# LiliMeng/network_interpretation_imagenet

Measured on AMD Instinct MI355X. Metric: masked-forward-passes/sec (224x224, resnet101), higher is better.
Workload: dtype f16x3 (split-fp16 MFMA, fp32 accumulate); stem conv in fp32 by superposition over superpixels; 1 GPU; resnet101, 512 masks/image x 128 images per GPU (BASELINE configs[2]; x1 GPUs); images_per_gpu=128, masks_per_image=512, forward_batch=2340, num_cus=256, entry=MaskedForwardEngine.score_packed, stem=table, lib_stamp=5d2f2b6c2eede968ac8309a9a3169fc2d6f530e9f9ea7d38be715b004f9c220a, lib_stamp_matches_tree=True, product_library=True, parallelism=mask-batch shard x1 + one all_gather of scores

## Files before the change

### include/mpx.h

```cpp
#ifndef MPX_H
#define MPX_H

#include <stddef.h>
#include <stdint.h>

#ifdef __cplusplus
extern "C" {
#endif

#define MPX_IMG 224
#define MPX_IMG_PAD 230
#define MPX_NUM_CLASSES 1000

enum {
    MPX_E_ARG = -1,
    MPX_E_STATE = -2,
    MPX_E_NOMEM = -3,
    MPX_E_INTERNAL = -4
};

#define MPX_ARCH_MNIST_NET 1
#define MPX_ARCH_CIFAR_RESNET 2000
#define MPX_ARCH_VGG 3000
#define MPX_ARCH_VGG_BN 3100
// ... 50 lines not shown
    int32_t hin;
    int32_t clamp_in;
} mpx_dwconv_desc;
int mpx_num_dwconvs(const mpx_engine* h);
int mpx_dwconv_info(const mpx_engine* h, int k, mpx_dwconv_desc* out);
int mpx_load_dwconv(mpx_engine* h, int k, const float* w, const float* gamma, const float* beta, const float* mean, const float* var, float eps);
int mpx_dwconv_params(const mpx_engine* h, int k, const float** w, const float** scale, const float** shift);

int mpx_set_conv_tile(mpx_engine* h, int i, int tile);
int mpx_get_conv_tile(const mpx_engine* h, int i);
int mpx_last_conv_kernels(const mpx_engine* h);

int mpx_pack_conv_weights(const mpx_conv_desc* d, const float* w, const float* conv_bias, const float* gamma,
                          const float* beta, const float* mean, const float* var, float eps,
                          uint16_t* w_hi, uint16_t* w_lo, float* scale, float* shift);
int mpx_mask_apply_normalize(mpx_engine* h, const uint8_t* img_u8_hwc, const float* img_f32_chw,
                             const int32_t* seg, const uint8_t* onoff, int M, int S,
                             const float mean[3], const float std[3], int slot0,
                             float* out_f32_nchw, void* stream);

int mpx_stem_table_build(mpx_engine* h, const uint8_t* img_u8_hwc, const float* img_f32_chw, const int32_t* seg, int S,
                         const float mean[3], const float std[3], void* stream);
int mpx_stem_table_apply(mpx_engine* h, const uint8_t* onoff, int M, int S, int slot0, void* stream);

int mpx_mask_apply_minmax(mpx_engine* h, const float* img_f32_chw, const int32_t* seg, const uint8_t* removed,
                          int M, int S, int slot0, float* out_f32_nchw, void* stream);

int mpx_avgpool2_pad(mpx_engine* h, const void* in_hi, const void* in_lo, void* out_hi, void* out_lo, int B,
                     int hin, int cin_p, int cout_p, void* stream);

int mpx_conv_bn_act(mpx_engine* h, int i, const void* in_hi, const void* in_lo,
                    const void* res_hi, const void* res_lo, void* out_hi, void* out_lo,
                    float* out_f32, int B, void* stream);

int mpx_conv_dual_bn_act(mpx_engine* h, int i, const void* in_hi, const void* in_lo, const void* x_hi,
                         const void* x_lo, void* out_hi, void* out_lo, int B, void* stream);
int mpx_set_fusion(mpx_engine* h, int mask);

int mpx_bottleneck_tail(mpx_engine* h, int i, const void* t1_hi, const void* t1_lo, const void* x_hi, const void* x_lo,
                        void* out_hi, void* out_lo, void* next_hi, void* next_lo, int B, void* stream);
int mpx_num_bottleneck_tails(const mpx_engine* h);
int mpx_bottleneck_tail_info(const mpx_engine* h, int k, int* conv2, int* conv3, int* downsample, int* next_conv1);

int mpx_maxpool3x3s2(mpx_engine* h, const void* in_hi, const void* in_lo, void* out_hi,
                     void* out_lo, int B, int hin, int c, void* stream);

// ... 60 lines not shown
```

### network_interpretation_imagenet_amd/_lib.py

```python
import ctypes as C
import os

import torch

_HERE = os.path.dirname(os.path.abspath(__file__))
PRODUCT_LIB_PATH = os.path.join(_HERE, "libmpx.so")
LIB_PATH = os.environ.get("MPX_LIB_PATH") or PRODUCT_LIB_PATH

IMG = 224
IMG_PAD = 230
NUM_CLASSES = 1000


class MpxError(RuntimeError):
    pass


class ConvDesc(C.Structure):
    _fields_ = [("name", C.c_char * 48), ("bn_name", C.c_char * 48),
                ("cin", C.c_int32), ("cout", C.c_int32), ("ksize", C.c_int32),
                ("stride", C.c_int32), ("pad", C.c_int32), ("hin", C.c_int32),
                ("hout", C.c_int32), ("relu", C.c_int32), ("residual", C.c_int32),
                ("k_packed", C.c_int32), ("cout_pad", C.c_int32)]

# ... 11 lines not shown
_fp = C.POINTER(C.c_float)

SIGNATURES = {
    "mpx_create": (_i, [_i, _i, _i, C.POINTER(_vp)]),
    "mpx_destroy": (_i, [_vp]),
    "mpx_last_error": (C.c_char_p, [_vp]),
    "mpx_max_batch": (_i, [_vp]),
    "mpx_num_cus": (_i, [_vp]),
    "mpx_workspace_bytes": (C.c_size_t, [_vp]),
    "mpx_num_convs": (_i, [_vp]),
    "mpx_conv_info": (_i, [_vp, _i, C.POINTER(ConvDesc)]),
    "mpx_set_conv_weights": (_i, [_vp, _i, _vp, _vp, _vp, _vp, _vp, _vp, _f]),
    "mpx_geometry": (_i, [_vp, C.POINTER(_i), C.POINTER(_i), C.POINTER(_i), C.POINTER(_i)]),
    "mpx_mask_apply_minmax": (_i, [_vp, _vp, _vp, _vp, _i, _i, _i, _vp, _vp]),
    "mpx_avgpool2_pad": (_i, [_vp, _vp, _vp, _vp, _vp, _i, _i, _i, _i, _vp]),
    "mpx_weights_complete": (_i, [_vp]),
    "mpx_set_conv_tile": (_i, [_vp, _i, _i]),
    "mpx_get_conv_tile": (_i, [_vp, _i]),
    "mpx_last_conv_kernels": (_i, [_vp]),
    "mpx_pack_conv_weights": (_i, [C.POINTER(ConvDesc), _vp, _vp, _vp, _vp, _vp, _vp, _f, _vp, _vp, _vp, _vp]),
    "mpx_mask_apply_normalize": (_i, [_vp, _vp, _vp, _vp, _vp, _i, _i, _fp, _fp, _i, _vp, _vp]),
    "mpx_stem_table_build": (_i, [_vp, _vp, _vp, _vp, _i, _fp, _fp, _vp]),
    "mpx_stem_table_apply": (_i, [_vp, _vp, _i, _i, _i, _vp]),
    "mpx_conv_bn_act": (_i, [_vp, _i, _vp, _vp, _vp, _vp, _vp, _vp, _vp, _i, _vp]),
    "mpx_conv_dual_bn_act": (_i, [_vp, _i, _vp, _vp, _vp, _vp, _vp, _vp, _i, _vp]),
    "mpx_set_fusion": (_i, [_vp, _i]),
    "mpx_bottleneck_tail": (_i, [_vp, _i, _vp, _vp, _vp, _vp, _vp, _vp, _vp, _vp, _i, _vp]),
    "mpx_num_bottleneck_tails": (_i, [_vp]),
    "mpx_bottleneck_tail_info": (_i, [_vp, _i, C.POINTER(_i), C.POINTER(_i), C.POINTER(_i), C.POINTER(_i)]),
    "mpx_stem_conv_maxpool": (_i, [_vp, _vp, _vp, _i, _vp]),
    "mpx_maxpool3x3s2": (_i, [_vp, _vp, _vp, _vp, _vp, _i, _i, _i, _vp]),
    "mpx_maxpool2x2s2": (_i, [_vp, _vp, _vp, _vp, _vp, _i, _i, _i, _vp]),
    "mpx_maxpool3x3s2p0": (_i, [_vp, _vp, _vp, _vp, _vp, _i, _i, _i, _vp]),
    "mpx_global_avgpool": (_i, [_vp, _vp, _vp, _vp, _vp, _i, _i, _i, _vp]),
    "mpx_head_softmax_gather": (_i, [_vp, _vp, _vp, _vp, _vp, _i, _vp]),
    "mpx_forward": (_i, [_vp, _vp, _vp, _vp, _vp, _i, _vp]),
    "mpx_heatmap_accumulate": (_i, [_vp, _vp, _vp, _vp, _vp, _i, _i, _vp, _vp]),
    "mpx_input_planes": (_i, [_vp, C.POINTER(_vp), C.POINTER(_vp)]),
    "mpx_mark_input_staged": (_i, [_vp, _i, _i]),
    "mpx_stem_planes": (_i, [_vp, C.POINTER(_vp), C.POINTER(_vp)]),
    "mpx_profile_enable": (_i, [_vp, _i]),
    "mpx_profile_collect": (_i, [_vp, C.POINTER(C.c_double), C.POINTER(C.c_longlong), C.POINTER(C.c_double)]),
    "mpx_flops_per_forward": (C.c_double, [_vp]),
    "mpx_num_norms": (_i, [_vp]),
    "mpx_norm_info": (_i, [_vp, _i, C.POINTER(NormDesc)]),
    "mpx_load_norm": (_i, [_vp, _i, _vp, _vp, _vp, _vp, _f]),
# ... 66 lines not shown
```

### network_interpretation_imagenet_amd/csrc/mpx_api.hip

```cpp
#include "../../include/mpx.h"
#include "mpx_kernels.h"
#include "mpx_conv3p.h"
#include "mpx_conv3pp.h"
#include "mpx_conv256.h"
#include "mpx_conv256p.h"
#include "mpx_convx.h"
#include "mpx_convw.h"
#include "mpx_btail.h"
#include "mpx_stemtab.h"
#include "mpx_dw.h"
#include "mpx_fire.h"
#include "mpx_pool3c.h"

#include <algorithm>
#include <cmath>
#include <cstdarg>
#include <initializer_list>
#include <new>
#include <cstdio>
#include <cstdlib>
#include <cstring>
#include <string>
#include <vector>

// ... 118 lines not shown
    char* arena = nullptr;
    size_t arena_bytes = 0;
    char* tab_arena = nullptr;
    size_t tab_arena_bytes = 0;
    half_t* in_hi = nullptr;
    half_t* in_lo = nullptr;
    half_t* act_hi[kActBufs] = {};
    half_t* act_lo[kActBufs] = {};
    half_t* pool_hi = nullptr;
    half_t* pool_lo = nullptr;
    float* logits = nullptr;
    float* seg_scratch = nullptr;
    half_t* stem_hi = nullptr;
    half_t* stem_lo = nullptr;
    float* stem_w32 = nullptr;
    float* stem_s32 = nullptr;
    float* stem_t32 = nullptr;
    int* tab_cnt = nullptr;
    int* tab_off = nullptr;
    int* tab_lab = nullptr;
    int* tab_heavy = nullptr;
    float* tab_vec = nullptr;
    unsigned* tab_bits = nullptr;
    size_t tab_sizes[4] = {0, 0, 0, 0};
    int tab_S = -1;
    bool stem_w_loaded = false;
    std::vector<uint8_t> slot_src;
    std::string err;
    bool in_forward = false;
    unsigned last_kernels = 0;
    bool fuse_ds = true;
    bool fuse_pool = true;
    bool prof_on = false;
    std::vector<ProfRec> prof_pool;
    int prof_used = 0;
    hipStream_t prof_stream = nullptr;
#ifdef MPX_DIAG
    unsigned long long* stamps = nullptr;
#endif
};

namespace {

int fail(mpx_engine* h, int code, const char* fmt, ...) {
    if (h) {
        char buf[512];
// ... 1683 lines not shown
    p.M = M; p.S = S; p.slot0 = slot0;
    p.size = MPX_IMG; p.pad_size = MPX_IMG_PAD; p.border = 3;
    MPX_SET_DEVICE(h);
    hipStream_t st = as_stream(stream);
    ProfScope ps(h, st, 1, -1);
    dim3 grid((MPX_IMG * MPX_IMG + 255) / 256, (M + K0_MT - 1) / K0_MT);
    hipLaunchKernelGGL(mask_apply_normalize_kernel, grid, dim3(256), lds, st, p);
    MPX_HIP(h, hipGetLastError());
    std::fill(h->slot_src.begin() + slot0, h->slot_src.begin() + slot0 + M, (uint8_t)1);
    return 0;
}

int mpx_stem_table_build(mpx_engine* h, const uint8_t* img_u8_hwc, const float* img_f32_chw, const int32_t* seg, int S,
                         const float mean[3], const float std[3], void* stream) {
    if (!h) return MPX_E_ARG;
    if (h->densenet) return fail(h, MPX_E_STATE, "stem_table_build: a DenseNet engine keeps no stem table; it stages through mpx_mask_apply_normalize");
    if (!h->stem_w32) return fail(h, MPX_E_STATE, "stem_table_build: this architecture has no 7x7 stem with a max pool%s", h->vgg || h->alexnet || h->mobilenet || h->squeezenet || h->googlenet ? " (VGG, AlexNet, MobileNetV2, SqueezeNet and GoogLeNet stage through mpx_mask_apply_normalize)" : "");
    if ((img_u8_hwc == nullptr) == (img_f32_chw == nullptr))
        return fail(h, MPX_E_ARG, "stem_table_build: exactly one of img_u8_hwc / img_f32_chw must be given");
    if (!seg || S <= 0 || S > 4096) return fail(h, MPX_E_ARG, "stem_table_build: null label map or S outside [1, 4096]");
    if (img_u8_hwc && (!mean || !std)) return fail(h, MPX_E_ARG, "stem_table_build: mean/std required for u8 input");
    if (!h->stem_w_loaded) return fail(h, MPX_E_STATE, "stem_table_build: layer 0 (%s) has no weights", h->convs[0].d.name);
    MPX_SET_DEVICE(h);
    if (!h->tab_arena) {
        const size_t total = 3 * h->tab_sizes[0] + h->tab_sizes[1] + h->tab_sizes[2] + h->tab_sizes[3];
        MPX_HIP(h, hipMalloc((void**)&h->tab_arena, total));
        h->tab_arena_bytes = total;
        char* cur = h->tab_arena;
        auto take = [&](size_t n) { char* r = cur; cur += n; return r; };
        h->tab_cnt = (int*)take(h->tab_sizes[0]);
        h->tab_off = (int*)take(h->tab_sizes[0]);
        h->tab_heavy = (int*)take(h->tab_sizes[0]);
        h->tab_lab = (int*)take(h->tab_sizes[1]);
        h->tab_vec = (float*)take(h->tab_sizes[2]);
        h->tab_bits = (unsigned*)take(h->tab_sizes[3]);
    }
    StemTabParams p;
    std::memset(&p, 0, sizeof p);
    p.img_u8 = img_u8_hwc; p.img_f32 = img_f32_chw; p.seg = seg; p.S = S;
    for (int c = 0; c < 3; ++c) {
        p.mean[c] = mean ? mean[c] : 0.f;
        p.std[c] = std ? std[c] : 1.f;
    }
    p.w = h->stem_w32; p.cnt = h->tab_cnt; p.off = h->tab_off; p.lab = h->tab_lab; p.vec = h->tab_vec;
    MPX_SET_DEVICE(h);
    hipStream_t st = as_stream(stream);
    ProfScope ps(h, st, 1, -1);
    hipLaunchKernelGGL(stemtab_count_kernel, dim3(ST_NPIX / 4), dim3(256), 0, st, p);
    MPX_HIP(h, hipGetLastError());
    hipLaunchKernelGGL(stemtab_scan_kernel, dim3(1), dim3(1024), 0, st, (const int*)h->tab_cnt, h->tab_off);
    MPX_HIP(h, hipGetLastError());
    hipLaunchKernelGGL(stemtab_fill_kernel, dim3(ST_NPIX / 4), dim3(256), 0, st, p);
    MPX_HIP(h, hipGetLastError());
    hipLaunchKernelGGL(stemtab_heavy_kernel, dim3(1), dim3(1024), 0, st, (const int*)h->tab_off, h->tab_heavy, h->tab_heavy + ST_POOLED * ST_POOLED);
    MPX_HIP(h, hipGetLastError());
    h->tab_S = S;
    return 0;
}

int mpx_stem_table_apply(mpx_engine* h, const uint8_t* onoff, int M, int S, int slot0, void* stream) {
    if (!h) return MPX_E_ARG;
    if (h->densenet) return fail(h, MPX_E_STATE, "stem_table_apply: a DenseNet engine keeps no stem table; it stages through mpx_mask_apply_normalize");
    if (!h->stem_w32) return fail(h, MPX_E_STATE, "stem_table_apply: this architecture has no 7x7 stem with a max pool");
    if (!onoff || M <= 0) return fail(h, MPX_E_ARG, "stem_table_apply: null mask rows or empty M");
    if (h->tab_S < 0) return fail(h, MPX_E_STATE, "stem_table_apply: no table in place (mpx_stem_table_build first; loading layer 0 again discards it)");
    if (S != h->tab_S) return fail(h, MPX_E_ARG, "stem_table_apply: S=%d, the table was built with S=%d", S, h->tab_S);
    if (slot0 < 0 || slot0 + M > h->max_batch) return fail(h, MPX_E_STATE, "stem_table_apply: slots [%d,%d) exceed max_batch %d", slot0, slot0 + M, h->max_batch);
    const int nmb = (M + 31) / 32;
    MPX_SET_DEVICE(h);
    hipStream_t st = as_stream(stream);
    {
        ProfScope ps(h, st, 1, -1);
        hipLaunchKernelGGL(onoff_bitplanes_kernel, dim3((S * nmb + 255) / 256), dim3(256), 0, st, onoff, M, S, nmb, h->tab_bits);
        MPX_HIP(h, hipGetLastError());
    }
    StemApplyParams p;
    std::memset(&p, 0, sizeof p);
    p.off = h->tab_off; p.lab = h->tab_lab; p.vec = h->tab_vec; p.bits = h->tab_bits; p.s = h->stem_s32; p.t = h->stem_t32;
    p.out_hi = h->stem_hi; p.out_lo = h->stem_lo; p.nmb = nmb; p.M = M; p.slot0 = slot0;
    p.heavy_list = h->tab_heavy; p.heavy_count = h->tab_heavy + ST_POOLED * ST_POOLED;
    {
        ProfScope ps(h, st, OP_CONV, 0);
        hipLaunchKernelGGL(stem_apply_heavy_kernel, dim3(h->num_cus, nmb), dim3(256), 0, st, p);
        MPX_HIP(h, hipGetLastError());
        hipLaunchKernelGGL(stem_apply_kernel, dim3(ST_POOLED * ST_POOLED / 4, nmb), dim3(256), 0, st, p);
        MPX_HIP(h, hipGetLastError());
    }
    std::fill(h->slot_src.begin() + slot0, h->slot_src.begin() + slot0 + M, (uint8_t)2);
    return 0;
}

int mpx_mask_apply_minmax(mpx_engine* h, const float* img_f32_chw, const int32_t* seg, const uint8_t* removed, int M, int S,
                          int slot0, float* out_f32_nchw, void* stream) {
    if (!h) return MPX_E_ARG;
    if (!h->small) return fail(h, MPX_E_STATE, "mask_apply_minmax: only the small networks (MNIST net, CIFAR ResNet) use this mask convention");
    if (!img_f32_chw || !seg || !removed || M <= 0 || S <= 0 || S > 4096) return fail(h, MPX_E_ARG, "mask_apply_minmax: null input, empty M/S or S > 4096");
    if (slot0 < 0 || slot0 + M > h->max_batch) return fail(h, MPX_E_STATE, "mask_apply_minmax: slots [%d,%d) exceed max_batch %d", slot0, slot0 + M, h->max_batch);
    MPX_SET_DEVICE(h);
    hipStream_t st = as_stream(stream);
    ProfScope ps(h, st, 1, -1);
    const int hw = h->img * h->img;
    float* stats = h->k0_scratch;
    float* mask_max = h->k0_scratch + 2 + 4096;
    hipLaunchKernelGGL(smallnet_image_stats_kernel, dim3(1), dim3(256), 0, st, img_f32_chw, seg, h->in_ch, hw, S, stats);
    MPX_HIP(h, hipGetLastError());
    hipLaunchKernelGGL(smallnet_mask_max_kernel, dim3((M + 255) / 256), dim3(256), 0, st, removed, M, S, (const float*)stats, mask_max);
    MPX_HIP(h, hipGetLastError());
    SmallMaskParams p;
// ... 394 lines not shown
                CatNormParams p;
                std::memset(&p, 0, sizeof p);
                p.f_hi = hi(o.in); p.f_lo = lo(o.in); p.r_hi = hi(o.res); p.r_lo = lo(o.res); p.y_hi = hi(o.out); p.y_lo = lo(o.out);
                p.scale = nl.scale; p.shift = nl.shift;
                p.npix = (long long)B * o.hin * o.hin;
                p.f_stride = o.g; p.c_total = o.ctot; p.c_old = o.c - o.g; p.c_begin = 0; p.c_end = o.c;
                rc = launch_catnorm(h, p, o.conv, as_stream(stream));
                break;
            }
        }
        if (rc) return rc;
    }
    return 0;
}

int mpx_stem_conv_maxpool(mpx_engine* h, void* out_hi, void* out_lo, int B, void* stream) {
    if (!h) return MPX_E_ARG;
    if (!out_hi || !out_lo || B <= 0) return fail(h, MPX_E_ARG, "stem + max pool: null pointer or empty batch");
    if (B > h->max_batch) return fail(h, MPX_E_STATE, "stem + max pool: B=%d exceeds max_batch=%d", B, h->max_batch);
    MPX_SET_DEVICE(h);
    return launch_stem_pool(h, (half_t*)out_hi, (half_t*)out_lo, B, as_stream(stream));
}

int mpx_set_fusion(mpx_engine* h, int mask) {
    if (!h) return MPX_E_ARG;
    h->fuse_pool = (mask & 1) != 0;
    h->fuse_ds = (mask & 1) != 0;
    h->fuse_bt = (mask & 2) != 0;
    return 0;
}

int mpx_bottleneck_tail(mpx_engine* h, int i, const void* t1_hi, const void* t1_lo, const void* x_hi, const void* x_lo,
                        void* out_hi, void* out_lo, void* next_hi, void* next_lo, int B, void* stream) {
    if (!h) return MPX_E_ARG;
    if (B <= 0 || (t1_hi == nullptr) != (t1_lo == nullptr) || !x_hi || !x_lo || !out_hi || !out_lo || !next_hi || !next_lo)
        return fail(h, MPX_E_ARG, "bottleneck_tail: null planes or empty batch");
    int ti = -1;
    for (size_t k = 0; k < h->tails.size(); ++k)
        if (h->tails[k].c2 == i) ti = (int)k;
    if (ti < 0) return fail(h, MPX_E_ARG, "bottleneck_tail: layer %d is not the conv2 of a block whose tail runs as one launch", i);
    {
        const TailBlock& tb = h->tails[ti];
        const size_t px = (size_t)B * h->convs[tb.c2].d.hin * h->convs[tb.c2].d.hin * sizeof(half_t);
        const size_t c_x = tb.ds >= 0 ? BT_MID : BT_OUT, c_next = (size_t)h->convs[tb.next1].d.cout;
        struct Range { const char* lo; size_t n; const char* what; };
        const Range r[8] = {{(const char*)t1_hi, px * BT_MID, "t1_hi"}, {(const char*)t1_lo, px * BT_MID, "t1_lo"},
// ... 147 lines not shown
```

### network_interpretation_imagenet_amd/csrc/mpx_stemtab.h

```cpp
#pragma once
#include "mpx_conv.h"

namespace mpx {

constexpr int ST_IN = 224, ST_CONV = 112, ST_POOLED = 56, ST_TAPS = 49, ST_C = 64;
constexpr int ST_NPIX = ST_CONV * ST_CONV;
constexpr int ST_MAX_ENTRIES = ST_NPIX * ST_TAPS;

struct StemTabParams {
    const uint8_t* img_u8;
    const float* img_f32;
    const int32_t* seg;
    float mean[3], std[3];
    int S;
    const float* w;
    int* cnt;
    int* off;
    int* lab;
    float* vec;
};

__device__ __forceinline__ int st_tap_label(const StemTabParams& p, int oy, int ox, int t, int* pix_out) {
    const int ky = t / 7, kx = t - ky * 7;
    const int iy = 2 * oy - 3 + ky, ix = 2 * ox - 3 + kx;
    if ((unsigned)iy >= (unsigned)ST_IN || (unsigned)ix >= (unsigned)ST_IN) return -1;
    const int pix = iy * ST_IN + ix;
    *pix_out = pix;
    const int l = p.seg[pix];
    return (unsigned)l < (unsigned)p.S ? l : -1;
}

__device__ __forceinline__ unsigned long long st_first_occurrences(const int* s_lab, int lane, int my_label) {
    bool first = lane < ST_TAPS && my_label >= 0;
    for (int t = 0; t < lane && t < ST_TAPS; ++t) first = first && (s_lab[t] != my_label);
    return __ballot(first);
}

__global__ __launch_bounds__(256) void stemtab_count_kernel(const StemTabParams p) {
    __shared__ int s_lab[4][64];
    const int lane = threadIdx.x & 63, wave = threadIdx.x >> 6;
    const int q = blockIdx.x * 4 + wave;
    const int oy = q / ST_CONV, ox = q - oy * ST_CONV;
    int pix = 0;
    const int l = lane < ST_TAPS ? st_tap_label(p, oy, ox, lane, &pix) : -1;
    s_lab[wave][lane] = l;
    __syncthreads();
    const unsigned long long firsts = st_first_occurrences(s_lab[wave], lane, l);
    if (lane == 0) p.cnt[q] = __popcll(firsts);
}

__global__ __launch_bounds__(1024) void stemtab_scan_kernel(const int* __restrict__ cnt, int* __restrict__ off) {
    __shared__ int s[1024];
    constexpr int PER = (ST_NPIX + 1023) / 1024;
    const int t = threadIdx.x, base = t * PER;
    int sum = 0;
    for (int i = 0; i < PER; ++i)
        if (base + i < ST_NPIX) sum += cnt[base + i];
    s[t] = sum;
    __syncthreads();
    for (int d = 1; d < 1024; d <<= 1) {
        const int v = t >= d ? s[t - d] : 0;
        __syncthreads();
        s[t] += v;
        __syncthreads();
    }
    int run = s[t] - sum;
    for (int i = 0; i < PER; ++i)
        if (base + i < ST_NPIX) {
            off[base + i] = run;
            run += cnt[base + i];
        }
    if (t == 1023) off[ST_NPIX] = s[1023];
}

__global__ __launch_bounds__(256) void stemtab_fill_kernel(const StemTabParams p) {
// ... 44 lines not shown
                                                              unsigned* __restrict__ bits) {
    const int i = blockIdx.x * 256 + threadIdx.x;
    if (i >= S * nmb) return;
    const int mb = i / S, s = i - mb * S;
    unsigned w = 0;
    for (int j = 0; j < 32; ++j) {
        const int m = mb * 32 + j;
        if (m < M && onoff[(size_t)m * S + s]) w |= 1u << j;
    }
    bits[(size_t)s * nmb + mb] = w;
}

struct StemApplyParams {
    const int* __restrict__ off;
    const int* __restrict__ lab;
    const float* __restrict__ vec;
    const unsigned* __restrict__ bits;
    const float* __restrict__ s;
    const float* __restrict__ t;
    half_t* __restrict__ out_hi;
    half_t* __restrict__ out_lo;
    const int* __restrict__ heavy_list;
    const int* __restrict__ heavy_count;
    int nmb, M, slot0;
};

__device__ __forceinline__ void stem_store4_packed(const StemApplyParams& p, unsigned (*s_out)[4][4][ST_C], int m, int mcount, int wave, int lane,
                                                   unsigned packed, size_t out0_row) {
    s_out[(m >> 2) & 1][m & 3][wave][lane] = packed;
    if ((m & 3) != 3 && m != mcount - 1) return;
    __syncthreads();
    const int ms = (m & ~3) + wave;
    if (ms < mcount) {
        typedef unsigned u4 __attribute__((ext_vector_type(4)));
        typedef unsigned u2 __attribute__((ext_vector_type(2)));
        const u4 q = *(const u4*)&s_out[(m >> 2) & 1][ms & 3][lane >> 4][(lane & 15) * 4];
        u2 vh, vl;
        vh[0] = (q[0] & 0xffffu) | (q[1] << 16);
        vh[1] = (q[2] & 0xffffu) | (q[3] << 16);
        vl[0] = (q[0] >> 16) | (q[1] & 0xffff0000u);
        vl[1] = (q[2] >> 16) | (q[3] & 0xffff0000u);
        const size_t o = out0_row + (size_t)ms * ST_POOLED * ST_POOLED * ST_C + (size_t)(lane >> 4) * ST_C + (lane & 15) * 4;
        __builtin_nontemporal_store(vh, (u2*)(p.out_hi + o));
        __builtin_nontemporal_store(vl, (u2*)(p.out_lo + o));
    }
}
// ... 30 lines not shown
                                                float (&R)[SA_CH], unsigned& starts, unsigned& kbv) {
    const int cnt = min(SA_CH, n_e - cb);
    starts = 0;
#pragma unroll
    for (int i = 0; i < SA_CH; ++i) {
        int g = 0;
        bool st = false;
        stem_entry(w, cb + i, g, st);
        const bool ok = i < cnt;
        R[i] = ok ? p.vec[(size_t)g * ST_C + lane] : 0.f;
        if (ok && st && cb + i > 0) starts |= 1u << i;
    }
    kbv = 0;
    if (lane < cnt) {
        int g = 0;
        bool st = false;
        stem_entry(w, cb + lane, g, st);
        kbv = p.bits[(size_t)p.lab[g] * p.nmb + mb];
    }
}

constexpr int SA_KF_PITCH = 56;

template <int KPP, bool BORDER>
__device__ __forceinline__ void stem_apply_fast(const StemApplyParams& p, unsigned (*s_out)[4][4][ST_C], float (*s_kf)[SA_KF_PITCH], int wave,
                                                int lane, int mcount, size_t out0_row, const int (&o)[9], const int (&len)[9],
                                                const bool (&qok)[9], float sc, float sh, int mb) {
    constexpr int NS = 9 * KPP, NS4 = (NS + 3) / 4 * 4;
    float R[NS4];
#pragma unroll
    for (int q = 0; q < 9; ++q)
#pragma unroll
        for (int k = 0; k < KPP; ++k) {
            const bool ok = k < len[q];
            const int g = o[q] + k;
            R[q * KPP + k] = ok ? p.vec[(size_t)g * ST_C + lane] : 0.f;
            const unsigned kb = ok ? p.bits[(size_t)p.lab[g] * p.nmb + mb] : 0u;
            if (lane < 32) s_kf[lane][q * KPP + k] = (kb >> lane & 1u) ? 1.0f : 0.0f;
        }
#pragma unroll
    for (int i = NS; i < NS4; ++i) {
        R[i] = 0.f;
        if (lane < 32) s_kf[lane][i] = 0.f;
    }
    __builtin_amdgcn_fence(__ATOMIC_RELEASE, "wavefront");
    __builtin_amdgcn_wave_barrier();
    __builtin_amdgcn_fence(__ATOMIC_ACQUIRE, "wavefront");
    for (int m = 0; m < mcount; ++m) {
        f4 kf[NS4 / 4];
#pragma unroll
        for (int i = 0; i < NS4 / 4; ++i) kf[i] = *(const f4*)&s_kf[m][4 * i];
        float best = -INFINITY;
#pragma unroll
        for (int q = 0; q < 9; ++q) {
            float v = 0.f;
#pragma unroll
            for (int k = 0; k < KPP; ++k)
                v = fmaf(kf[(q * KPP + k) / 4][(q * KPP + k) % 4], R[q * KPP + k], v);
            const float y = fmaxf(fmaf(v, sc, sh), 0.f);
            best = fmaxf(best, BORDER ? (qok[q] ? y : -INFINITY) : y);
        }
        stem_store4(p, s_out, m, mcount, wave, lane, best, out0_row);
    }
}

struct StemPixel {
    StemRows w;
    int n_e, n_empty, kmax;
    int o9[9], len9[9];
    bool qok[9];
    bool interior;
};

__device__ __forceinline__ void stem_pixel(const StemApplyParams& p, int py, int px, StemPixel& g) {
    const int cx0 = max(2 * px - 1, 0);
    const int ncol = 2 * px + 1 - cx0 + 1;
    StemRows& w = g.w;
    g.n_empty = 0;
    {
        const int cy0 = 2 * py - 1, cy1 = 2 * py, cy2 = 2 * py + 1;
        const bool ok0 = cy0 >= 0;
        const int q0 = (ok0 ? cy0 : 0) * ST_CONV + cx0, q1 = cy1 * ST_CONV + cx0, q2 = cy2 * ST_CONV + cx0;
        const int e00 = p.off[q0], e01 = p.off[q0 + 1], e02 = p.off[q0 + 2], e03 = p.off[q0 + ncol];
        const int e10 = p.off[q1], e11 = p.off[q1 + 1], e12 = p.off[q1 + 2], e13 = p.off[q1 + ncol];
        const int e20 = p.off[q2], e21 = p.off[q2 + 1], e22 = p.off[q2 + 2], e23 = p.off[q2 + ncol];
// ... 9 lines not shown
    const int e0[4] = {w.o00, w.o01, w.o02, w.a0 + w.l0}, e1[4] = {w.o10, w.o11, w.o12, w.a1 + w.l1}, e2[4] = {w.o20, w.o21, w.o22, w.a2 + w.l2};
    g.kmax = 0;
#pragma unroll
    for (int c = 0; c < 3; ++c) {
        const bool cok = col0_ok || c > 0;
        const int j = cok ? (col0_ok ? c : c - 1) : 0;
        g.qok[c] = cok && row0_ok;
        g.qok[3 + c] = cok;
        g.qok[6 + c] = cok;
        g.o9[c] = e0[j];
        g.o9[3 + c] = e1[j];
        g.o9[6 + c] = e2[j];
        g.len9[c] = g.qok[c] ? e0[j + 1] - e0[j] : 0;
        g.len9[3 + c] = cok ? e1[j + 1] - e1[j] : 0;
        g.len9[6 + c] = cok ? e2[j + 1] - e2[j] : 0;
    }
#pragma unroll
    for (int q = 0; q < 9; ++q) g.kmax = max(g.kmax, g.len9[q]);
    g.interior = col0_ok && row0_ok;
}

__device__ __forceinline__ bool stem_heavy(const StemPixel& g) { return !(g.kmax <= 6 && (g.kmax <= 4 || g.interior)); }

__global__ __launch_bounds__(1024) void stemtab_heavy_kernel(const int* __restrict__ off, int* __restrict__ heavy_list, int* __restrict__ heavy_count) {
    __shared__ int s_n;
    if (threadIdx.x == 0) s_n = 0;
    __syncthreads();
    StemApplyParams p;
    p.off = off;
    for (int P = threadIdx.x; P < ST_POOLED * ST_POOLED; P += 1024) {
        StemPixel g;
        stem_pixel(p, P / ST_POOLED, P % ST_POOLED, g);
        if (stem_heavy(g)) heavy_list[atomicAdd(&s_n, 1)] = P;
    }
    __syncthreads();
    if (threadIdx.x == 0) *heavy_count = s_n;
}

__global__ __launch_bounds__(256) void stem_apply_heavy_kernel(const StemApplyParams p) {
    __shared__ __attribute__((aligned(16))) float s_ks[4][SA_MG * SA_CH];
    const int lane = threadIdx.x & 63;
    const int wave = __builtin_amdgcn_readfirstlane(threadIdx.x >> 6);
    const int mb = blockIdx.y;
    const int mw0 = wave * SA_MG;
    const int mcount = min(SA_MG, p.M - (mb * 32 + mw0));
    if (mcount <= 0) return;
// ... 41 lines not shown
                        }
                        v[k] = fmaf(kf[ii], R[i], v[k]);
                    }
                }
            }
        }
    }
    const size_t out0 = (((size_t)(p.slot0 + mb * 32 + mw0) * ST_POOLED + py) * ST_POOLED + px) * ST_C + lane;
#pragma unroll
    for (int k = 0; k < SA_MG; ++k) {
        if (k < mcount) {
            const float b = g.n_e > 0 ? fmaxf(best[k], fmaxf(fmaf(v[k], sc, sh), 0.f)) : best[k];
            half_t hi, lo;
            split_f32(b, hi, lo);
            const size_t o = out0 + (size_t)k * ST_POOLED * ST_POOLED * ST_C;
            p.out_hi[o] = hi;
            p.out_lo[o] = lo;
        }
    }
    __builtin_amdgcn_wave_barrier();
  }
}

__global__ __launch_bounds__(256) void stem_apply_kernel(const StemApplyParams p) {
    __shared__ __attribute__((aligned(16))) unsigned s_out[2][4][4][ST_C];
    __shared__ __attribute__((aligned(16))) float s_kf[4][32][SA_KF_PITCH];
    const int lane = threadIdx.x & 63;
    const int wave = __builtin_amdgcn_readfirstlane(threadIdx.x >> 6);
    const int P = blockIdx.x * 4 + wave;
    const int mb = blockIdx.y;
    const int m0 = mb * 32;
    const int mcount = min(32, p.M - m0);
    const int py = P / ST_POOLED, px = P - py * ST_POOLED;
    StemPixel g;
    stem_pixel(p, py, px, g);
    const float sc = p.s[lane], sh = p.t[lane];
    const size_t out0_row = (((size_t)(p.slot0 + m0) * ST_POOLED + py) * ST_POOLED + (px - wave)) * ST_C;
    if (stem_heavy(g)) {
        const size_t o0 = out0_row + (size_t)wave * ST_C + lane;
        for (int m = 0; m < mcount; ++m) {
            const size_t o = o0 + (size_t)m * ST_POOLED * ST_POOLED * ST_C;
            const unsigned packed = (unsigned)__builtin_bit_cast(unsigned short, p.out_hi[o]) | ((unsigned)__builtin_bit_cast(unsigned short, p.out_lo[o]) << 16);
            stem_store4_packed(p, s_out, m, mcount, wave, lane, packed, out0_row);
        }
    } else if (g.interior) {
        if (g.kmax <= 1) stem_apply_fast<1, false>(p, s_out, s_kf[wave], wave, lane, mcount, out0_row, g.o9, g.len9, g.qok, sc, sh, mb);
        else if (g.kmax <= 2) stem_apply_fast<2, false>(p, s_out, s_kf[wave], wave, lane, mcount, out0_row, g.o9, g.len9, g.qok, sc, sh, mb);
        else if (g.kmax <= 3) stem_apply_fast<3, false>(p, s_out, s_kf[wave], wave, lane, mcount, out0_row, g.o9, g.len9, g.qok, sc, sh, mb);
        else if (g.kmax <= 4) stem_apply_fast<4, false>(p, s_out, s_kf[wave], wave, lane, mcount, out0_row, g.o9, g.len9, g.qok, sc, sh, mb);
        else stem_apply_fast<6, false>(p, s_out, s_kf[wave], wave, lane, mcount, out0_row, g.o9, g.len9, g.qok, sc, sh, mb);
    } else {
        if (g.kmax <= 2) stem_apply_fast<2, true>(p, s_out, s_kf[wave], wave, lane, mcount, out0_row, g.o9, g.len9, g.qok, sc, sh, mb);
        else stem_apply_fast<4, true>(p, s_out, s_kf[wave], wave, lane, mcount, out0_row, g.o9, g.len9, g.qok, sc, sh, mb);
    }
}

}
```

### network_interpretation_imagenet_amd/engine.py

```python
import ctypes as C

import numpy as np
import torch

from . import _lib
from ._lib import MpxError, IMG, NUM_CLASSES

MEAN = (0.485, 0.456, 0.406)
STD = (0.229, 0.224, 0.225)
BN_EPS = 1e-5
GOOGLENET_BN_EPS = 1e-3

ARCH_IDS = {"resnet18": 18, "resnet34": 34, "resnet50": 50, "resnet101": 101, "resnet152": 152,
            "mnist_net": 1, "cifar_resnet20": 2020, "cifar_resnet56": 2056, "cifar_resnet110": 2110}
ARCH_IDS.update({"vgg%d%s" % (d, bn): (3100 if bn else 3000) + d for d in (11, 13, 16, 19) for bn in ("", "_bn")})
ARCH_IDS["alexnet"] = 4000
ARCH_IDS.update({"densenet%d" % d: 5000 + d for d in (121, 169, 201)})
ARCH_IDS["mobilenet_v2"] = 6002
ARCH_IDS["squeezenet1_1"] = 7011
ARCH_IDS["googlenet"] = 8000


COMPUTE_UNITS = 256
ROUND_PIXELS_14 = 256
# ... 525 lines not shown
        labels = torch.full((m,), int(label), dtype=torch.int32, device=self.device)
        self.score_packed([self._image_to_device(image)], seg_d, [onoff_d], labels, score, pred, stem=stem)
        self.heatmap_accumulate(seg_d, onoff_d, pred, labels, buf[:IMG * IMG].view(IMG, IMG))
        buf[IMG * IMG] += (pred == labels).sum()
        return score, pred

    def heatmap(self, seg_rank, onoff, pred, label):
        m = int(np.asarray(onoff).shape[0])
        heat = torch.zeros(IMG, IMG, dtype=torch.float32, device=self.device)
        if m:
            t = lambda a, dt: torch.from_numpy(np.ascontiguousarray(a, dtype=dt)).to(self.device)
            self.heatmap_accumulate(t(seg_rank, np.int32), t(onoff, np.uint8), t(pred, np.int32),
                                    torch.full((m,), int(label), dtype=torch.int32, device=self.device), heat)
        return heat.cpu().numpy().astype(np.float64)

    def set_conv_tile(self, layer, tile):
        i = layer if isinstance(layer, int) else [d.name.decode() for d in self.layers].index(layer)
        _lib.check(self._h, self._lib.mpx_set_conv_tile(self._h, int(i), int(tile)), "mpx_set_conv_tile")

    def set_fusion(self, on=True):
        mask = (3 if on else 0) if isinstance(on, bool) else int(on)
        _lib.check(self._h, self._lib.mpx_set_fusion(self._h, mask), "mpx_set_fusion")

    def bottleneck_tails(self):
        out = []
        for k in range(self._lib.mpx_num_bottleneck_tails(self._h)):
            v = [C.c_int() for _ in range(4)]
            _lib.check(self._h, self._lib.mpx_bottleneck_tail_info(self._h, k, *[C.byref(x) for x in v]), "mpx_bottleneck_tail_info")
            out.append(tuple(int(x.value) for x in v))
        return out

    def conv_tile(self, layer):
        i = layer if isinstance(layer, int) else [d.name.decode() for d in self.layers].index(layer)
        return int(self._lib.mpx_get_conv_tile(self._h, int(i)))

    def profile(self, on=True):
        _lib.check(self._h, self._lib.mpx_profile_enable(self._h, 1 if on else 0), "mpx_profile_enable")

    def collect_profile(self):
        ms = (C.c_double * 4)()
        n = (C.c_longlong * 4)()
        per = (C.c_double * len(self.layers))()
        per_norm = (C.c_double * max(1, len(self.norms)))()
        avg2 = (C.c_double * 1)()
        per_dw = (C.c_double * max(1, len(self.dwconvs)))()
        n_cp = int(self._lib.mpx_num_clip_pools(self._h))
# ... 7 lines not shown
```

Baseline: 23270 masked-forward-passes/s.

## Precompute stem outputs for all superpixel on/off combos and gather per mask

When the table is built, each pooled stem pixel covered by at most four superpixels gets every one of its 2^n possible on/off outputs precomputed and stored as packed hi/lo fp16. At apply time, groups where all four pixels qualify skip the per-mask superposition and only index the precomputed row with each mask's bits, then stream it out. This swaps per-mask arithmetic for a small per-image precompute plus memory gathers, at the cost of extra table memory, an extra build kernel and extra grid rows in the apply launch.

```diff
diff --git a/include/mpx.h b/include/mpx.h
--- a/include/mpx.h
+++ b/include/mpx.h
@@ -96,6 +96,8 @@
 int mpx_stem_table_build(mpx_engine* h, const uint8_t* img_u8_hwc, const float* img_f32_chw, const int32_t* seg, int S,
                          const float mean[3], const float std[3], void* stream);
 int mpx_stem_table_apply(mpx_engine* h, const uint8_t* onoff, int M, int S, int slot0, void* stream);
+int mpx_set_stem_combos(mpx_engine* h, int on);
+int mpx_stem_combo_counts(mpx_engine* h, int* eligible, int* served, void* stream);
 
 int mpx_mask_apply_minmax(mpx_engine* h, const float* img_f32_chw, const int32_t* seg, const uint8_t* removed,
                           int M, int S, int slot0, float* out_f32_nchw, void* stream);
diff --git a/network_interpretation_imagenet_amd/_lib.py b/network_interpretation_imagenet_amd/_lib.py
--- a/network_interpretation_imagenet_amd/_lib.py
+++ b/network_interpretation_imagenet_amd/_lib.py
@@ -57,6 +57,8 @@
     "mpx_mask_apply_normalize": (_i, [_vp, _vp, _vp, _vp, _vp, _i, _i, _fp, _fp, _i, _vp, _vp]),
     "mpx_stem_table_build": (_i, [_vp, _vp, _vp, _vp, _i, _fp, _fp, _vp]),
     "mpx_stem_table_apply": (_i, [_vp, _vp, _i, _i, _i, _vp]),
+    "mpx_set_stem_combos": (_i, [_vp, _i]),
+    "mpx_stem_combo_counts": (_i, [_vp, C.POINTER(_i), C.POINTER(_i), _vp]),
     "mpx_conv_bn_act": (_i, [_vp, _i, _vp, _vp, _vp, _vp, _vp, _vp, _vp, _i, _vp]),
     "mpx_conv_dual_bn_act": (_i, [_vp, _i, _vp, _vp, _vp, _vp, _vp, _vp, _i, _vp]),
     "mpx_set_fusion": (_i, [_vp, _i]),
diff --git a/network_interpretation_imagenet_amd/csrc/mpx_api.hip b/network_interpretation_imagenet_amd/csrc/mpx_api.hip
--- a/network_interpretation_imagenet_amd/csrc/mpx_api.hip
+++ b/network_interpretation_imagenet_amd/csrc/mpx_api.hip
@@ -164,6 +164,15 @@
     int* tab_heavy = nullptr;
     float* tab_vec = nullptr;
     unsigned* tab_bits = nullptr;
+    unsigned* tab_combo = nullptr;
+    int* tab_combo_lab = nullptr;
+    int* tab_combo_info = nullptr;
+    bool tab_has_combos = false;
+#ifndef MPX_PROBE_NO_STEM_COMBOS
+    bool stem_combos = true;
+#else
+    bool stem_combos = false;
+#endif
     size_t tab_sizes[4] = {0, 0, 0, 0};
     int tab_S = -1;
     bool stem_w_loaded = false;
@@ -1893,8 +1902,11 @@
     if (img_u8_hwc && (!mean || !std)) return fail(h, MPX_E_ARG, "stem_table_build: mean/std required for u8 input");
     if (!h->stem_w_loaded) return fail(h, MPX_E_STATE, "stem_table_build: layer 0 (%s) has no weights", h->convs[0].d.name);
     MPX_SET_DEVICE(h);
+    const size_t combo_bytes = round_up((size_t)ST_POOLED * ST_POOLED * SC_PITCH * ST_C * 4, 256);
+    const size_t combo_lab_bytes = round_up((size_t)ST_POOLED * ST_POOLED * SC_MAXLAB * 4, 256);
+    const size_t combo_info_bytes = round_up((size_t)(ST_NGROUPS + 2) * 4, 256);
     if (!h->tab_arena) {
-        const size_t total = 3 * h->tab_sizes[0] + h->tab_sizes[1] + h->tab_sizes[2] + h->tab_sizes[3];
+        const size_t total = 3 * h->tab_sizes[0] + h->tab_sizes[1] + h->tab_sizes[2] + h->tab_sizes[3] + combo_bytes + combo_lab_bytes + combo_info_bytes;
         MPX_HIP(h, hipMalloc((void**)&h->tab_arena, total));
         h->tab_arena_bytes = total;
         char* cur = h->tab_arena;
@@ -1905,6 +1917,9 @@
         h->tab_lab = (int*)take(h->tab_sizes[1]);
         h->tab_vec = (float*)take(h->tab_sizes[2]);
         h->tab_bits = (unsigned*)take(h->tab_sizes[3]);
+        h->tab_combo = (unsigned*)take(combo_bytes);
+        h->tab_combo_lab = (int*)take(combo_lab_bytes);
+        h->tab_combo_info = (int*)take(combo_info_bytes);
     }
     StemTabParams p;
     std::memset(&p, 0, sizeof p);
@@ -1919,11 +1934,22 @@
     ProfScope ps(h, st, 1, -1);
     hipLaunchKernelGGL(stemtab_count_kernel, dim3(ST_NPIX / 4), dim3(256), 0, st, p);
     MPX_HIP(h, hipGetLastError());
-    hipLaunchKernelGGL(stemtab_scan_kernel, dim3(1), dim3(1024), 0, st, (const int*)h->tab_cnt, h->tab_off);
+    h->tab_has_combos = h->stem_combos;
+    int* const heavy_count = h->tab_heavy + ST_POOLED * ST_POOLED;
+    hipLaunchKernelGGL(stemtab_scan_kernel, dim3(1), dim3(1024), 0, st, (const int*)h->tab_cnt, h->tab_off,
+                       h->tab_has_combos ? heavy_count : nullptr, h->tab_has_combos ? h->tab_combo_info + ST_NGROUPS : nullptr);
     MPX_HIP(h, hipGetLastError());
     hipLaunchKernelGGL(stemtab_fill_kernel, dim3(ST_NPIX / 4), dim3(256), 0, st, p);
     MPX_HIP(h, hipGetLastError());
-    hipLaunchKernelGGL(stemtab_heavy_kernel, dim3(1), dim3(1024), 0, st, (const int*)h->tab_off, h->tab_heavy, h->tab_heavy + ST_POOLED * ST_POOLED);
+    if (h->tab_has_combos) {
+        StemApplyParams a;
+        std::memset(&a, 0, sizeof a);
+        a.off = h->tab_off; a.lab = h->tab_lab; a.vec = h->tab_vec; a.s = h->stem_s32; a.t = h->stem_t32;
+        hipLaunchKernelGGL(stemtab_combos_kernel, dim3(ST_NGROUPS), dim3(256), 0, st, a, h->tab_combo, h->tab_combo_lab, h->tab_combo_info,
+                           h->tab_heavy, heavy_count);
+    } else {
+        hipLaunchKernelGGL(stemtab_heavy_kernel, dim3(1), dim3(1024), 0, st, (const int*)h->tab_off, h->tab_heavy, heavy_count);
+    }
     MPX_HIP(h, hipGetLastError());
     h->tab_S = S;
     return 0;
@@ -1950,11 +1976,15 @@
     p.off = h->tab_off; p.lab = h->tab_lab; p.vec = h->tab_vec; p.bits = h->tab_bits; p.s = h->stem_s32; p.t = h->stem_t32;
     p.out_hi = h->stem_hi; p.out_lo = h->stem_lo; p.nmb = nmb; p.M = M; p.slot0 = slot0;
     p.heavy_list = h->tab_heavy; p.heavy_count = h->tab_heavy + ST_POOLED * ST_POOLED;
+    const bool gather = h->stem_combos && h->tab_has_combos;
+    if (gather) {
+        p.combo = h->tab_combo; p.combo_lab = h->tab_combo_lab; p.served = h->tab_combo_info;
+    }
     {
         ProfScope ps(h, st, OP_CONV, 0);
         hipLaunchKernelGGL(stem_apply_heavy_kernel, dim3(h->num_cus, nmb), dim3(256), 0, st, p);
         MPX_HIP(h, hipGetLastError());
-        hipLaunchKernelGGL(stem_apply_kernel, dim3(ST_POOLED * ST_POOLED / 4, nmb), dim3(256), 0, st, p);
+        hipLaunchKernelGGL(stem_apply_kernel, dim3(ST_NGROUPS, nmb + (gather ? (nmb + SG_MB - 1) / SG_MB : 0)), dim3(256), 0, st, p);
         MPX_HIP(h, hipGetLastError());
     }
     std::fill(h->slot_src.begin() + slot0, h->slot_src.begin() + slot0 + M, (uint8_t)2);
@@ -2395,6 +2425,27 @@
     return launch_stem_pool(h, (half_t*)out_hi, (half_t*)out_lo, B, as_stream(stream));
 }
 
+int mpx_set_stem_combos(mpx_engine* h, int on) {
+    if (!h) return MPX_E_ARG;
+    h->stem_combos = on != 0;
+    return 0;
+}
+
+int mpx_stem_combo_counts(mpx_engine* h, int* eligible, int* served, void* stream) {
+    if (!h || !eligible || !served) return MPX_E_ARG;
+    if (h->tab_S < 0) return fail(h, MPX_E_STATE, "stem_combo_counts: no table in place (mpx_stem_table_build first)");
+    int n[2] = {0, 0};
+    if (h->tab_has_combos) {
+        MPX_SET_DEVICE(h);
+        hipStream_t st = as_stream(stream);
+        MPX_HIP(h, hipMemcpyAsync(n, h->tab_combo_info + ST_NGROUPS, sizeof n, hipMemcpyDeviceToHost, st));
+        MPX_HIP(h, hipStreamSynchronize(st));
+    }
+    *eligible = n[0];
+    *served = n[1];
+    return 0;
+}
+
 int mpx_set_fusion(mpx_engine* h, int mask) {
     if (!h) return MPX_E_ARG;
     h->fuse_pool = (mask & 1) != 0;
diff --git a/network_interpretation_imagenet_amd/csrc/mpx_stemtab.h b/network_interpretation_imagenet_amd/csrc/mpx_stemtab.h
--- a/network_interpretation_imagenet_amd/csrc/mpx_stemtab.h
+++ b/network_interpretation_imagenet_amd/csrc/mpx_stemtab.h
@@ -6,6 +6,8 @@
 constexpr int ST_IN = 224, ST_CONV = 112, ST_POOLED = 56, ST_TAPS = 49, ST_C = 64;
 constexpr int ST_NPIX = ST_CONV * ST_CONV;
 constexpr int ST_MAX_ENTRIES = ST_NPIX * ST_TAPS;
+constexpr int ST_NGROUPS = ST_POOLED * ST_POOLED / 4;
+constexpr int SC_MAXLAB = 4, SC_PITCH = 1 << SC_MAXLAB;
 
 struct StemTabParams {
     const uint8_t* img_u8;
@@ -49,8 +51,11 @@
     if (lane == 0) p.cnt[q] = __popcll(firsts);
 }
 
-__global__ __launch_bounds__(1024) void stemtab_scan_kernel(const int* __restrict__ cnt, int* __restrict__ off) {
+__global__ __launch_bounds__(1024) void stemtab_scan_kernel(const int* __restrict__ cnt, int* __restrict__ off, int* __restrict__ heavy_count,
+                                                            int* __restrict__ combo_counts) {
     __shared__ int s[1024];
+    if (heavy_count && threadIdx.x == 0) *heavy_count = 0;
+    if (combo_counts && threadIdx.x < 2) combo_counts[threadIdx.x] = 0;
     constexpr int PER = (ST_NPIX + 1023) / 1024;
     const int t = threadIdx.x, base = t * PER;
     int sum = 0;
@@ -141,6 +146,9 @@
     half_t* __restrict__ out_lo;
     const int* __restrict__ heavy_list;
     const int* __restrict__ heavy_count;
+    const unsigned* __restrict__ combo;
+    const int* __restrict__ combo_lab;
+    const int* __restrict__ served;
     int nmb, M, slot0;
 };
 
@@ -217,10 +225,10 @@
 
 constexpr int SA_KF_PITCH = 56;
 
-template <int KPP, bool BORDER>
-__device__ __forceinline__ void stem_apply_fast(const StemApplyParams& p, unsigned (*s_out)[4][4][ST_C], float (*s_kf)[SA_KF_PITCH], int wave,
-                                                int lane, int mcount, size_t out0_row, const int (&o)[9], const int (&len)[9],
-                                                const bool (&qok)[9], float sc, float sh, int mb) {
+template <int KPP, bool BORDER, class Bits, class Store>
+__device__ __forceinline__ void stem_apply_fast(const StemApplyParams& p, float (*s_kf)[SA_KF_PITCH], int lane, int mcount,
+                                                const int (&o)[9], const int (&len)[9], const bool (&qok)[9], float sc, float sh,
+                                                Bits bits, Store store) {
     constexpr int NS = 9 * KPP, NS4 = (NS + 3) / 4 * 4;
     float R[NS4];
 #pragma unroll
@@ -230,7 +238,7 @@
             const bool ok = k < len[q];
             const int g = o[q] + k;
             R[q * KPP + k] = ok ? p.vec[(size_t)g * ST_C + lane] : 0.f;
-            const unsigned kb = ok ? p.bits[(size_t)p.lab[g] * p.nmb + mb] : 0u;
+            const unsigned kb = ok ? bits(g) : 0u;
             if (lane < 32) s_kf[lane][q * KPP + k] = (kb >> lane & 1u) ? 1.0f : 0.0f;
         }
 #pragma unroll
@@ -255,7 +263,7 @@
             const float y = fmaxf(fmaf(v, sc, sh), 0.f);
             best = fmaxf(best, BORDER ? (qok[q] ? y : -INFINITY) : y);
         }
-        stem_store4(p, s_out, m, mcount, wave, lane, best, out0_row);
+        store(m, best);
     }
 }
 
@@ -311,6 +319,21 @@
 
 __device__ __forceinline__ bool stem_heavy(const StemPixel& g) { return !(g.kmax <= 6 && (g.kmax <= 4 || g.interior)); }
 
+template <class Bits, class Store>
+__device__ __forceinline__ void stem_apply_static(const StemApplyParams& p, float (*s_kf)[SA_KF_PITCH], int lane, int mcount, const StemPixel& g,
+                                                  float sc, float sh, Bits bits, Store store) {
+    if (g.interior) {
+        if (g.kmax <= 1) stem_apply_fast<1, false>(p, s_kf, lane, mcount, g.o9, g.len9, g.qok, sc, sh, bits, store);
+        else if (g.kmax <= 2) stem_apply_fast<2, false>(p, s_kf, lane, mcount, g.o9, g.len9, g.qok, sc, sh, bits, store);
+        else if (g.kmax <= 3) stem_apply_fast<3, false>(p, s_kf, lane, mcount, g.o9, g.len9, g.qok, sc, sh, bits, store);
+        else if (g.kmax <= 4) stem_apply_fast<4, false>(p, s_kf, lane, mcount, g.o9, g.len9, g.qok, sc, sh, bits, store);
+        else stem_apply_fast<6, false>(p, s_kf, lane, mcount, g.o9, g.len9, g.qok, sc, sh, bits, store);
+    } else {
+        if (g.kmax <= 2) stem_apply_fast<2, true>(p, s_kf, lane, mcount, g.o9, g.len9, g.qok, sc, sh, bits, store);
+        else stem_apply_fast<4, true>(p, s_kf, lane, mcount, g.o9, g.len9, g.qok, sc, sh, bits, store);
+    }
+}
+
 __global__ __launch_bounds__(1024) void stemtab_heavy_kernel(const int* __restrict__ off, int* __restrict__ heavy_list, int* __restrict__ heavy_count) {
     __shared__ int s_n;
     if (threadIdx.x == 0) s_n = 0;
@@ -398,9 +421,123 @@
   }
 }
 
+__global__ __launch_bounds__(256) void stemtab_combos_kernel(const StemApplyParams p, unsigned* __restrict__ combo, int* __restrict__ combo_lab,
+                                                             int* __restrict__ info, int* __restrict__ heavy_list, int* __restrict__ heavy_count) {
+    __shared__ __attribute__((aligned(16))) float s_kf[4][32][SA_KF_PITCH];
+    __shared__ int s_elig[4];
+    const int lane = threadIdx.x & 63;
+    const int wave = __builtin_amdgcn_readfirstlane(threadIdx.x >> 6);
+    const int P = blockIdx.x * 4 + wave;
+    const int py = P / ST_POOLED, px = P - py * ST_POOLED;
+    StemPixel g;
+    stem_pixel(p, py, px, g);
+    if (lane == 0 && stem_heavy(g)) heavy_list[atomicAdd(heavy_count, 1)] = P;
+    int my = -1, l0 = -1, l1 = -1, l2 = -1, l3 = -1, n = SC_MAXLAB + 1;
+    if (g.kmax <= SC_MAXLAB) {
+        n = 0;
+        int o = 0, len = 0;
+#pragma unroll
+        for (int q = 0; q < 9; ++q)
+            if ((lane >> 2) == q) {
+                o = g.o9[q];
+                len = g.len9[q];
+            }
+        if (lane < 9 * SC_MAXLAB && (lane & 3) < len) my = p.lab[o + (lane & 3)];
+        unsigned long long rest = __ballot(my >= 0);
+        while (rest && n <= SC_MAXLAB) {
+            const int l = __builtin_amdgcn_readlane(my, __ffsll((long long)rest) - 1);
+            if (n == 0) l0 = l;
+            else if (n == 1) l1 = l;
+            else if (n == 2) l2 = l;
+            else if (n == 3) l3 = l;
+            ++n;
+            rest &= ~__ballot(my == l);
+        }
+    }
+    const bool eligible = n <= SC_MAXLAB;
+    if (lane == 0) s_elig[wave] = eligible;
+    if (eligible) {
+        if (lane < 4) combo_lab[P * 4 + lane] = lane == 0 ? l0 : (lane == 1 ? l1 : (lane == 2 ? l2 : l3));
+        unsigned* rows = combo + (size_t)P * SC_PITCH * ST_C + lane;
+        stem_apply_static(p, s_kf[wave], lane, 1 << n, g, p.s[lane], p.t[lane],
+                          [&](int e) {
+                              const int l = p.lab[e];
+                              return l == l0 ? 0xAAAAu : (l == l1 ? 0xCCCCu : (l == l2 ? 0xF0F0u : 0xFF00u));
+                          },
+                          [&](int c, float best) {
+                              half_t hi, lo;
+                              split_f32(best, hi, lo);
+                              rows[c * ST_C] = (unsigned)__builtin_bit_cast(unsigned short, hi) | ((unsigned)__builtin_bit_cast(unsigned short, lo) << 16);
+                          });
+    }
+    __syncthreads();
+    if (threadIdx.x == 0) {
+        const int ne = s_elig[0] + s_elig[1] + s_elig[2] + s_elig[3];
+        info[blockIdx.x] = ne == 4;
+        if (ne > 0) atomicAdd(&info[ST_NGROUPS], ne);
+        if (ne == 4) atomicAdd(&info[ST_NGROUPS + 1], 4);
+    }
+}
+
+constexpr int SG_MB = 4;
+
+__device__ __forceinline__ void stem_apply_gather(const StemApplyParams& p, int group, int gy, unsigned (*s_combo)[SC_PITCH][ST_C]) {
+    typedef unsigned u4 __attribute__((ext_vector_type(4)));
+    typedef int i4 __attribute__((ext_vector_type(4)));
+    const int lane = threadIdx.x & 63;
+    const int wave = __builtin_amdgcn_readfirstlane(threadIdx.x >> 6);
+    const int P0 = group * 4;
+    {
+        const i4 L = *(const i4*)(p.combo_lab + (P0 + wave) * 4);
+        const int rows = 1 << ((L[0] >= 0) + (L[1] >= 0) + (L[2] >= 0) + (L[3] >= 0));
+        const u4* src = (const u4*)(p.combo + (size_t)(P0 + wave) * SC_PITCH * ST_C);
+        u4* dst = (u4*)&s_combo[wave][0][0];
+        for (int i = lane; i < rows * (ST_C / 4); i += 64) dst[i] = src[i];
+    }
+    const int pw = (lane >> 3) & 3, half = lane >> 5;
+    const i4 L = *(const i4*)(p.combo_lab + (P0 + pw) * 4);
+    const unsigned* mine = &s_combo[pw][0][(lane & 7) * 8];
+    __syncthreads();
+    for (int mbi = 0; mbi < SG_MB; ++mbi) {
+        const int mb = gy * SG_MB + mbi;
+        if (mb >= p.nmb) break;
+        unsigned bw[SC_MAXLAB];
+#pragma unroll
+        for (int k = 0; k < SC_MAXLAB; ++k) bw[k] = L[k] >= 0 ? p.bits[(size_t)L[k] * p.nmb + mb] : 0u;
+#pragma unroll
+        for (int it = 0; it < 4; ++it) {
+            const int j = it * 8 + wave * 2 + half;
+            const int m = mb * 32 + j;
+            if (m >= p.M) continue;
+            int c = 0;
+#pragma unroll
+            for (int k = 0; k < SC_MAXLAB; ++k) c |= (int)(bw[k] >> j & 1u) << k;
+            const u4 a = *(const u4*)(mine + c * ST_C), b = *(const u4*)(mine + c * ST_C + 4);
+            u4 vh, vl;
+            vh[0] = (a[0] & 0xffffu) | (a[1] << 16);
+            vh[1] = (a[2] & 0xffffu) | (a[3] << 16);
+            vh[2] = (b[0] & 0xffffu) | (b[1] << 16);
+            vh[3] = (b[2] & 0xffffu) | (b[3] << 16);
+            vl[0] = (a[0] >> 16) | (a[1] & 0xffff0000u);
+            vl[1] = (a[2] >> 16) | (a[3] & 0xffff0000u);
+            vl[2] = (b[0] >> 16) | (b[1] & 0xffff0000u);
+            vl[3] = (b[2] >> 16) | (b[3] & 0xffff0000u);
+            const size_t o = ((size_t)(p.slot0 + m) * ST_POOLED * ST_POOLED + P0) * ST_C + (lane & 31) * 8;
+            __builtin_nontemporal_store(vh, (u4*)(p.out_hi + o));
+            __builtin_nontemporal_store(vl, (u4*)(p.out_lo + o));
+        }
+    }
+}
+
+
 __global__ __launch_bounds__(256) void stem_apply_kernel(const StemApplyParams p) {
     __shared__ __attribute__((aligned(16))) unsigned s_out[2][4][4][ST_C];
     __shared__ __attribute__((aligned(16))) float s_kf[4][32][SA_KF_PITCH];
+    if ((int)blockIdx.y >= p.nmb) {
+        if (p.served[blockIdx.x]) stem_apply_gather(p, blockIdx.x, blockIdx.y - p.nmb, (unsigned (*)[SC_PITCH][ST_C])s_kf);
+        return;
+    }
+    const int served = p.served ? p.served[blockIdx.x] : 0;
     const int lane = threadIdx.x & 63;
     const int wave = __builtin_amdgcn_readfirstlane(threadIdx.x >> 6);
     const int P = blockIdx.x * 4 + wave;
@@ -411,6 +548,7 @@
     StemPixel g;
     stem_pixel(p, py, px, g);
     const float sc = p.s[lane], sh = p.t[lane];
+    if (served) return;
     const size_t out0_row = (((size_t)(p.slot0 + m0) * ST_POOLED + py) * ST_POOLED + (px - wave)) * ST_C;
     if (stem_heavy(g)) {
         const size_t o0 = out0_row + (size_t)wave * ST_C + lane;
@@ -419,16 +557,11 @@
             const unsigned packed = (unsigned)__builtin_bit_cast(unsigned short, p.out_hi[o]) | ((unsigned)__builtin_bit_cast(unsigned short, p.out_lo[o]) << 16);
             stem_store4_packed(p, s_out, m, mcount, wave, lane, packed, out0_row);
         }
-    } else if (g.interior) {
-        if (g.kmax <= 1) stem_apply_fast<1, false>(p, s_out, s_kf[wave], wave, lane, mcount, out0_row, g.o9, g.len9, g.qok, sc, sh, mb);
-        else if (g.kmax <= 2) stem_apply_fast<2, false>(p, s_out, s_kf[wave], wave, lane, mcount, out0_row, g.o9, g.len9, g.qok, sc, sh, mb);
-        else if (g.kmax <= 3) stem_apply_fast<3, false>(p, s_out, s_kf[wave], wave, lane, mcount, out0_row, g.o9, g.len9, g.qok, sc, sh, mb);
-        else if (g.kmax <= 4) stem_apply_fast<4, false>(p, s_out, s_kf[wave], wave, lane, mcount, out0_row, g.o9, g.len9, g.qok, sc, sh, mb);
-        else stem_apply_fast<6, false>(p, s_out, s_kf[wave], wave, lane, mcount, out0_row, g.o9, g.len9, g.qok, sc, sh, mb);
     } else {
-        if (g.kmax <= 2) stem_apply_fast<2, true>(p, s_out, s_kf[wave], wave, lane, mcount, out0_row, g.o9, g.len9, g.qok, sc, sh, mb);
-        else stem_apply_fast<4, true>(p, s_out, s_kf[wave], wave, lane, mcount, out0_row, g.o9, g.len9, g.qok, sc, sh, mb);
-    }
-}
-
-}
+        stem_apply_static(p, s_kf[wave], lane, mcount, g, sc, sh,
+                          [&](int e) { return p.bits[(size_t)p.lab[e] * p.nmb + mb]; },
+                          [&](int m, float best) { stem_store4(p, s_out, m, mcount, wave, lane, best, out0_row); });
+    }
+}
+
+}
diff --git a/network_interpretation_imagenet_amd/engine.py b/network_interpretation_imagenet_amd/engine.py
--- a/network_interpretation_imagenet_amd/engine.py
+++ b/network_interpretation_imagenet_amd/engine.py
@@ -571,6 +571,14 @@
         mask = (3 if on else 0) if isinstance(on, bool) else int(on)
         _lib.check(self._h, self._lib.mpx_set_fusion(self._h, mask), "mpx_set_fusion")
 
+    def set_stem_combos(self, on=True):
+        _lib.check(self._h, self._lib.mpx_set_stem_combos(self._h, 1 if on else 0), "mpx_set_stem_combos")
+
+    def stem_combo_counts(self):
+        e, v = C.c_int(), C.c_int()
+        _lib.check(self._h, self._lib.mpx_stem_combo_counts(self._h, C.byref(e), C.byref(v), self._stream()), "mpx_stem_combo_counts")
+        return int(e.value), int(v.value)
+
     def bottleneck_tails(self):
         out = []
         for k in range(self._lib.mpx_num_bottleneck_tails(self._h)):
```

Result: no change. 23430 masked-forward-passes/s (median of 6 runs) (+0.7%).
